# LongmaoTeamTf/deep_recommenders

Hardware: AMD Instinct MI355X
Metric: examples/sec/node DeepFM (26 sparse feats, 10M vocab, dim 64) (higher is better)
Workload: dtype f32; 1 GPU; DeepFM Criteo-shape synthetic training step (BASELINE.json configs[2]): 26 sparse + 13 dense, 10000000 vocab/field hashed on device, dim 64, DNN [256, 32]+[1] relu, sigmoid-CE, fused SGD; batch 65536 per GPU, ids uniform; tables on one GPU (66.6 GB); gemm_split=f16x2, global_batch=65536, parallelism=single, per_kernel_events=False

## Files before the change

deep_recommenders_amd/csrc/bf3_wgrad.hip:

```cpp
#ifndef DR_NT_WGRAD_GATHER
#define DR_NT_WGRAD_GATHER 0
#endif
#include "bf3_rs_core.h"

namespace {

using namespace drrs;

struct TnRsArgs {
    const float* X; int64_t ldx;
    const float* Y; int64_t ldy;
    int64_t R; int32_t F; int32_t N;
    int64_t per; int32_t split;
    float* partial; float* colsum;
    const int32_t* ids_t; const int64_t* row_base; const float* table; int32_t nf; const float* dense_pad;
    const uint32_t* x_amax; const uint32_t* x2_amax; const uint32_t* y_amax;
};

template <int GATHER, int H2 = 0>
__global__ __launch_bounds__(512, 2) void bf3_gemm_tn_rs_kernel(TnRsArgs g) {
    constexpr int NW = 8, BMF = 32 * NW, BN = 256, NT = BN / 32;
    constexpr int NPL = RS_NPL<H2>, B_PLANE = RS_B_PLANE, STAGE = RS_STAGE<H2>;
    __shared__ __attribute__((aligned(1024))) unsigned char smem[2 * STAGE];

    const int tid = threadIdx.x, lane = tid & 63;
    const int wave = __builtin_amdgcn_readfirstlane(tid >> 6);
    const int l31 = lane & 31, hi = lane >> 5;
    const int tiles_n = (g.N + BN - 1) / BN, tiles_f = (g.F + BMF - 1) / BMF;
    const int per_slice = tiles_f * tiles_n;
    const int Fp = tiles_f * BMF, Np = tiles_n * BN;
    const int lid = xcd_remap(blockIdx.x, per_slice * g.split);
    const int slice = lid / per_slice, t = lid % per_slice;
    const int f0 = (t / tiles_n) * BMF, n0 = (t % tiles_n) * BN;
    const int64_t r_begin = (int64_t)slice * g.per;
    int64_t r_end = r_begin + g.per;
    if (r_end > g.R) r_end = g.R;
    const int nk = (int)((r_end - r_begin + BK - 1) / BK);
    const bool want_cs = g.colsum != nullptr && f0 == 0;
    float h2_sx = 1.f, h2_sy = 1.f;
    if constexpr (H2) {
        float inv;
        h2_prologue(g.x_amax, g.x2_amax, g.y_amax, h2_sx, h2_sy, inv);
    }

    const int fcol = min(f0 + wave * 32 + l31, g.F - 1);
    const int ncol = min(n0 + wave * 32 + l31, g.N - 1);
    const unsigned lds0 = (unsigned)(uintptr_t)(lds_ptr_t)smem;
    const int sw = tn_img_swizzle(l31);
    unsigned b_addr[2];
#pragma unroll
    for (int s = 0; s < 2; ++s) b_addr[s] = rs_frag_addr(lds0, l31, hi, sw, s);
    unsigned char* const wrow = smem + (wave * 32 + l31) * 64;

    float xa[16], yb[16];
    const unsigned xoff = (unsigned)((16 * hi * g.ldx + fcol) * 4), yoff = (unsigned)((16 * hi * g.ldy + ncol) * 4);
    auto load_raw = [&](float (&dst)[16], const float* base, int64_t ld, unsigned voff, int64_t r0) {
        if (r0 + BK <= r_end) {
// ... 219 lines not shown
    }
}

void launch_tn_rs_reduce(const float* partial, const float* colsum, int split, int32_t F, int32_t N, int Fp, int Np, float scale,
                         float* dst, int64_t ld, float* dstb, const uint32_t* x_amax, const uint32_t* x2_amax, const uint32_t* y_amax,
                         dr_stream_t stream) {
    const bool vec = ((reinterpret_cast<uintptr_t>(partial) | reinterpret_cast<uintptr_t>(dst)) & 15) == 0 && (ld & 3) == 0;
    if (vec)
        hipLaunchKernelGGL(bf3_tn_rs_reduce_kernel<4>, dim3(F, (N + 255) / 256), dim3(64), 0, dr_s(stream), partial, colsum, split, F, N,
                           Fp, Np, scale, dst, ld, dstb, x_amax, x2_amax, y_amax);
    else
        hipLaunchKernelGGL(bf3_tn_rs_reduce_kernel<1>, dim3(F, (N + 63) / 64), dim3(64), 0, dr_s(stream), partial, colsum, split, F, N,
                           Fp, Np, scale, dst, ld, dstb, x_amax, x2_amax, y_amax);
}

void tn_rs_plan(int64_t R, int32_t F, int32_t N, int& split, int64_t& per, int& Fp, int& Np) {
    const int tf = (F + 255) / 256, tn = (N + 255) / 256;
    Fp = tf * 256;
    Np = tn * 256;
    int64_t sp = 256 / ((int64_t)tf * tn);
    const int64_t max_split = (R + 16 * BK - 1) / (16 * BK);
    if (sp > max_split) sp = max_split;
    if (sp < 1) sp = 1;
    per = ((R + sp - 1) / sp + BK - 1) / BK * BK;
    split = (int)((R + per - 1) / per);
}
}

extern "C" int64_t dr_bf3_wgrad_workspace_bytes(int64_t R, int32_t F, int32_t N) {
    if (R <= 0 || F <= 0 || N <= 0) return 0;
// ... 3 lines not shown
    return ((int64_t)split * Fp * Np + (int64_t)split * Np) * (int64_t)sizeof(float);
}

static int wgrad_impl(const float* x, int64_t ld_x, const float* dy, int64_t ld_dy, int64_t R, int32_t F, int32_t N,
                      float scale, float* dstW, int64_t ld_w, float* dstb, void* workspace, int64_t workspace_bytes,
                      dr_stream_t stream, const uint32_t* x_amax = nullptr, const uint32_t* dy_amax = nullptr) {
    if (R <= 0 || F <= 0 || N <= 0) return DR_EINVAL;
    if (!x || !dy || !dstW || !workspace || ld_x < F || ld_dy < N || ld_w < N) return DR_EINVAL;
    if (workspace_bytes < dr_bf3_wgrad_workspace_bytes(R, F, N)) return DR_EINVAL;
    int split, Fp, Np;
    int64_t per;
    tn_rs_plan(R, F, N, split, per, Fp, Np);
    float* partial = static_cast<float*>(workspace);
    float* colsum = partial + (int64_t)split * Fp * Np;
    TnRsArgs g{x, ld_x, dy, ld_dy, R, F, N, per, split, partial, dstb != nullptr ? colsum : nullptr, nullptr, nullptr, nullptr, 0, nullptr,
               x_amax, nullptr, dy_amax};
    const int grid = (Fp / 256) * (Np / 256) * split;
    if (x_amax != nullptr) hipLaunchKernelGGL((bf3_gemm_tn_rs_kernel<0, 1>), dim3(grid), dim3(512), 0, dr_s(stream), g);
    else hipLaunchKernelGGL((bf3_gemm_tn_rs_kernel<0, 0>), dim3(grid), dim3(512), 0, dr_s(stream), g);
    launch_tn_rs_reduce(partial, dstb != nullptr ? colsum : nullptr, split, F, N, Fp, Np, scale, dstW, ld_w, dstb, x_amax, nullptr, dy_amax,
                        stream);
    DR_CHECK_LAUNCH();
    return DR_OK;
}

extern "C" int dr_bf3_wgrad(const float* x, int64_t ld_x, const float* dy, int64_t ld_dy, int64_t R, int32_t F, int32_t N,
                            float scale, float* dstW, int64_t ld_w, float* dstb, void* workspace, int64_t workspace_bytes,
                            dr_stream_t stream) {
    return wgrad_impl(x, ld_x, dy, ld_dy, R, F, N, scale, dstW, ld_w, dstb, workspace, workspace_bytes, stream);
}

extern "C" int dr_h2_wgrad(const float* x, int64_t ld_x, const uint32_t* x_amax, const float* dy, int64_t ld_dy, const uint32_t* dy_amax,
                           int64_t R, int32_t F, int32_t N, float scale, float* dstW, int64_t ld_w, float* dstb, void* workspace,
                           int64_t workspace_bytes, dr_stream_t stream) {
    if (!x_amax || !dy_amax) return DR_EINVAL;
    return wgrad_impl(x, ld_x, dy, ld_dy, R, F, N, scale, dstW, ld_w, dstb, workspace, workspace_bytes, stream, x_amax, dy_amax);
}

static int wgrad_emb_impl(const int32_t* ids_t, int64_t R, int32_t nf, const int64_t* row_base, const float* table, int32_t D,
                          const float* dense_pad, const float* dy, int64_t ld_dy, int32_t F, int32_t N, float scale, float* dstW,
                          int64_t ld_w, float* dstb, void* workspace, int64_t workspace_bytes, int32_t parts, dr_stream_t stream,
                          const uint32_t* table_amax = nullptr, const uint32_t* dense_amax = nullptr, const uint32_t* dy_amax = nullptr) {
    if (R <= 0 || F <= 0 || N <= 0 || nf <= 0) return DR_EINVAL;
    if (table_amax != nullptr && (!dy_amax || (F > 64 * nf && !dense_amax))) return DR_EINVAL;
    if (D != 64 || F < 64 * nf || F > 64 * nf + 32) return DR_ESHAPE;
    if (!ids_t || !row_base || !table || !dy || !dstW || !workspace || ld_dy < N || ld_w < N) return DR_EINVAL;
    if (F > 64 * nf && !dense_pad) return DR_EINVAL;
    if (workspace_bytes < dr_bf3_wgrad_workspace_bytes(R, F, N)) return DR_EINVAL;
    int split, Fp, Np;
    int64_t per;
    tn_rs_plan(R, F, N, split, per, Fp, Np);
    float* partial = static_cast<float*>(workspace);
    float* colsum = partial + (int64_t)split * Fp * Np;
    TnRsArgs g{nullptr, 0, dy, ld_dy, R, F, N, per, split, partial, dstb != nullptr ? colsum : nullptr, ids_t, row_base, table, nf,
               F > 64 * nf ? dense_pad : nullptr, table_amax, F > 64 * nf ? dense_amax : nullptr, dy_amax};
    const int grid = (Fp / 256) * (Np / 256) * split;
    if (parts & 1) {
        if (table_amax != nullptr) hipLaunchKernelGGL((bf3_gemm_tn_rs_kernel<1, 1>), dim3(grid), dim3(512), 0, dr_s(stream), g);
        else hipLaunchKernelGGL((bf3_gemm_tn_rs_kernel<1, 0>), dim3(grid), dim3(512), 0, dr_s(stream), g);
    }
    if (parts & 2)
        launch_tn_rs_reduce(partial, dstb != nullptr ? colsum : nullptr, split, F, N, Fp, Np, scale, dstW, ld_w, dstb, table_amax,
                            F > 64 * nf ? dense_amax : nullptr, dy_amax, stream);
    DR_CHECK_LAUNCH();
    return DR_OK;
}

extern "C" int dr_bf3_wgrad_emb(const int32_t* ids_t, int64_t R, int32_t nf, const int64_t* row_base, const float* table, int32_t D,
                                const float* dense_pad, const float* dy, int64_t ld_dy, int32_t F, int32_t N, float scale, float* dstW,
                                int64_t ld_w, float* dstb, void* workspace, int64_t workspace_bytes, int32_t parts, dr_stream_t stream) {
    if (parts < 1 || parts > 3) return DR_EINVAL;
    return wgrad_emb_impl(ids_t, R, nf, row_base, table, D, dense_pad, dy, ld_dy, F, N, scale, dstW, ld_w, dstb, workspace, workspace_bytes,
                          parts, stream);
}

extern "C" int dr_h2_wgrad_emb(const int32_t* ids_t, int64_t R, int32_t nf, const int64_t* row_base, const float* table, int32_t D,
                               const uint32_t* table_amax, const float* dense_pad, const uint32_t* dense_amax, const float* dy, int64_t ld_dy,
                               const uint32_t* dy_amax, int32_t F, int32_t N, float scale, float* dstW, int64_t ld_w, float* dstb,
                               void* workspace, int64_t workspace_bytes, int32_t parts, dr_stream_t stream) {
    if (parts < 1 || parts > 3 || !table_amax || !dy_amax) return DR_EINVAL;
    return wgrad_emb_impl(ids_t, R, nf, row_base, table, D, dense_pad, dy, ld_dy, F, N, scale, dstW, ld_w, dstb, workspace, workspace_bytes,
                          parts, stream, table_amax, dense_amax, dy_amax);
}
```

deep_recommenders_amd/csrc/h2_occ.hip:

```cpp
#include "dr_common.h"
#include "rs_args.h"
#include <algorithm>
#include <cstdlib>

namespace drrs {
namespace {

typedef _Float16 f16x4 __attribute__((ext_vector_type(4)));
typedef float f32x4 __attribute__((ext_vector_type(4)));
typedef float f32x16 __attribute__((ext_vector_type(16)));
typedef unsigned u32x4 __attribute__((ext_vector_type(4)));
typedef __attribute__((address_space(3))) void* lds_ptr_t;

#define OCC_DS_READ_B128(dst, addr, off) asm volatile("ds_read_b128 %0, %1 offset:%2" : "=v"(dst) : "v"(addr), "n"(off))
#define OCC_DS_WRITE_B64(addr, val, off) asm volatile("ds_write_b64 %0, %1 offset:%2" ::"v"(addr), "v"(val), "n"(off) : "memory")
#define OCC_DS_WRITE_B32(addr, val, off) asm volatile("ds_write_b32 %0, %1 offset:%2" ::"v"(addr), "v"(val), "n"(off) : "memory")

constexpr int BM = 256, BN = 256, BK = 32;
constexpr int PLANE = 256 * 64;
constexpr int A_OFF = 0, B_OFF = 2 * PLANE, STAGE = 4 * PLANE;

struct K4Args {
    const int32_t* ids_t;
    const uint8_t* flags;
    const int64_t* row_base; int32_t F;
    float* table; float* lin_w;
    const float* lin_old_t;
    const float* sum_x; const float* d_fm_logit;
    float scale;
    float* d_concat; int64_t ld_dc;
    uint32_t* table_amax;
};

template <int EPI, int DBG = 0>
__global__ __launch_bounds__(1024) void h2_occ_nt_kernel(RsArgs g, K4Args e) {
    __shared__ __attribute__((aligned(1024))) unsigned char smem[2 * STAGE + (EPI == 8 ? 10240 : 0)];

    const int tid = threadIdx.x, lane = tid & 63;
    const int wave = __builtin_amdgcn_readfirstlane(tid >> 6);
    const int l31 = lane & 31, hi = lane >> 5;
    const int wr = wave >> 2, wc = wave & 3;

    const int tiles_n = (g.N + BN - 1) / BN;
    const int tiles_m = (int)((g.M + BM - 1) / BM);
    const int ntiles = tiles_m * tiles_n;
    const int nk = (g.K + BK - 1) / BK;
    const bool ktail = (g.K % BK) != 0;
// ... 380 lines not shown
    }
}


constexpr int PM = 128;
constexpr int PA_PLANE = PM * 64, PB_PLANE = BN * 64;
constexpr int PA_OFF = 0, PB_OFF = 2 * PA_PLANE, PSTAGE = 2 * PA_PLANE + 2 * PB_PLANE;
constexpr int P_SXP = 2 * PSTAGE;
constexpr int P_STQ = P_SXP + PM * 256;
constexpr int P_DLP = P_STQ + 8 * 2048;
constexpr int P_LOP = P_DLP + PM * 4;
constexpr int P_UIP = P_LOP + 8 * 256;
constexpr int P_LDS = P_UIP + 8 * 256;
constexpr int P_EPI_BARRIERS = 7;

__global__ __launch_bounds__(1024) void h2_occ_pp_kernel(RsArgs g, K4Args e) {
    __shared__ __attribute__((aligned(1024))) unsigned char smem[P_LDS];

    const int tid = threadIdx.x, lane = tid & 63;
    const int wave = __builtin_amdgcn_readfirstlane(tid >> 6);
    const int grp = wave >> 3, wg = wave & 7;
    const int wr = wg >> 2, wc = wg & 3;

    const int tiles_n = (g.N + BN - 1) / BN;
    const int tiles_m = (int)((g.M + PM - 1) / PM);
    const int ntiles = tiles_m * tiles_n;
    const int nk = (g.K + BK - 1) / BK;
    const bool ktail = (g.K % BK) != 0;
    const int kv4 = (g.K + 3) / 4 * 4;
    const int nb = max(nk + 1, P_EPI_BARRIERS);

// ... 260 lines not shown
#pragma unroll
            for (int a = 0; a < 2; ++a)
#pragma unroll
                for (int b = 0; b < 2; ++b)
#pragma unroll
                    for (int reg = 0; reg < 16; ++reg) acc[a][b][reg] = 0.f;
        }
        bar();
        asm volatile("s_waitcnt vmcnt(0)" ::: "memory");
        bar();
        for (int b = P_EPI_BARRIERS; b < nb; ++b) bar();
    };

    const int n = (int)blockIdx.x < ntiles ? (ntiles - 1 - (int)blockIdx.x) / (int)gridDim.x + 1 : 0;
    auto idle = [&]() __attribute__((always_inline)) { for (int b = 0; b < nb; ++b) bar(); };
    if (grp == 1) idle();
    for (int i = grp; i < n; i += 2) {
        main_loop(i);
        epilogue(i);
    }
    if (((n ^ grp) & 1) == 0) idle();
    if (e.table_amax != nullptr) {
        uint32_t m = __float_as_uint(cmax);
#pragma unroll
        for (int o = 32; o > 0; o >>= 1) m = max(m, (uint32_t)__shfl_xor((int)m, o, 64));
        if (lane == 0 && m > __hip_atomic_load(e.table_amax, __ATOMIC_RELAXED, __HIP_MEMORY_SCOPE_AGENT)) atomicMax(e.table_amax, m);
    }
}

}

// ... 25 lines not shown
    }
#endif
    if (g.mask != nullptr) hipLaunchKernelGGL((h2_occ_nt_kernel<1>), dim3(grid), dim3(1024), 0, stream, g, K4Args{});
    else if (g.accumulate) hipLaunchKernelGGL((h2_occ_nt_kernel<3>), dim3(grid), dim3(1024), 0, stream, g, K4Args{});
    else hipLaunchKernelGGL((h2_occ_nt_kernel<0>), dim3(grid), dim3(1024), 0, stream, g, K4Args{});
    DR_CHECK_LAUNCH();
    return DR_OK;
}

}

extern "C" int dr_h2_dgrad_emb_sgd(const float* dy, int64_t ld_dy, const uint32_t* dy_amax, const void* w_planes, int64_t w_ps,
                                   int64_t w_ld, const uint32_t* w_amax, int64_t M, int32_t F, int32_t K, const int32_t* ids_t,
                                   const uint8_t* unique_flags, const int64_t* row_base, float* table, float* lin_w,
                                   const float* lin_old_t, const float* sum_x, const float* d_fm_logit, float scale, float* d_concat,
                                   int64_t ld_dconcat, uint32_t* table_amax, dr_stream_t stream) {
    using namespace drrs;
    if (M < 0 || F <= 0 || F > 64 || K <= 0 || !dy_amax || !w_amax) return DR_EINVAL;
    if (M == 0) return DR_OK;
    if (!dy || !w_planes || !ids_t || !unique_flags || !row_base || !table || !sum_x || !d_fm_logit || !d_concat) return DR_EINVAL;
    if ((lin_w != nullptr) != (lin_old_t != nullptr)) return DR_EINVAL;
    if ((reinterpret_cast<uintptr_t>(dy) & 15) != 0 || (ld_dy & 3) != 0 || ld_dy < K) return DR_EINVAL;
    if ((reinterpret_cast<uintptr_t>(w_planes) & 15) != 0 || w_ld < (K + BK - 1) / BK * BK || (w_ld & 7) != 0 || (w_ps & 7) != 0) return DR_EINVAL;
    if ((reinterpret_cast<uintptr_t>(d_concat) & 15) != 0 || (ld_dconcat & 3) != 0 || ld_dconcat < 64 * (int64_t)F) return DR_EINVAL;
    if ((reinterpret_cast<uintptr_t>(table) & 15) != 0 || (reinterpret_cast<uintptr_t>(sum_x) & 15) != 0) return DR_EINVAL;
    if (2 * w_ps * 2 + (int64_t)BK * 2 * ((K + BK - 1) / BK) > 0x7fffffffll) return DR_ESHAPE;
    if ((int64_t)(BM + 8) * ld_dy * 4 + (int64_t)K * 4 > 0x7fffffffll) return DR_ESHAPE;
    RsArgs g{};
    g.A = dy; g.lda = ld_dy; g.B = static_cast<const __bf16*>(w_planes); g.b_ps = w_ps; g.b_ld = w_ld;
    g.M = M; g.N = 64 * F; g.K = K;
    g.a_amax = dy_amax; g.b_amax = w_amax;
    K4Args e{ids_t, unique_flags, row_base, F, table, lin_w, lin_old_t, sum_x, d_fm_logit, scale, d_concat, ld_dconcat, table_amax};
    static const bool overlap = [] { const char* v = getenv("DR_FUSED_K4_OVERLAP"); return !(v && v[0] == '0' && v[1] == 0); }();
    const int64_t tiles = ((M + (overlap ? PM : BM) - 1) / (overlap ? PM : BM)) * ((g.N + BN - 1) / BN);
    if (tiles > 0x7fffffff) return DR_EINVAL;
    const int grid = (int)(tiles < 256 ? tiles : 256);
#ifdef DR_OCC_ABLATE
    {
        static const int dbg = [] { const char* v = getenv("DR_OCC_DBG"); return v ? atoi(v) : 0; }();
        if (dbg == 1024 || dbg == 2048) {
            const int grid8 = (int)std::min<int64_t>(((M + BM - 1) / BM) * ((g.N + BN - 1) / BN), 256);
            if (dbg == 1024) hipLaunchKernelGGL((h2_occ_nt_kernel<8, 1024>), dim3(grid8), dim3(1024), 0, dr_s(stream), g, e);
            else hipLaunchKernelGGL((h2_occ_nt_kernel<8, 2048>), dim3(grid8), dim3(1024), 0, dr_s(stream), g, e);
            DR_CHECK_LAUNCH();
            return DR_OK;
        }
    }
#endif
    if (overlap) hipLaunchKernelGGL(h2_occ_pp_kernel, dim3(grid), dim3(1024), 0, dr_s(stream), g, e);
    else hipLaunchKernelGGL((h2_occ_nt_kernel<8>), dim3(grid), dim3(1024), 0, dr_s(stream), g, e);
    DR_CHECK_LAUNCH();
    return DR_OK;
}
```

deep_recommenders_amd/csrc/rs_args.h:

```cpp
#pragma once
#include "dr_common.h"

namespace drrs {

__device__ __forceinline__ int xcd_remap(int bid, int nwg) {
    const int q = nwg / 8, r = nwg % 8;
    const int xcd = bid % 8, idx = bid / 8;
    return (xcd < r ? xcd * (q + 1) : r * (q + 1) + (xcd - r) * q) + idx;
}

struct RsArgs {
    const float* A; int64_t lda;
    const __bf16* B; int64_t b_ps, b_ld;
    int64_t M; int32_t N; int32_t K;
    float* C; int64_t ldc;
    const float* bias; int32_t act;
    const float* mask; int64_t ld_mask;
    int32_t accumulate;
    const float* x0; const float* xin; int64_t ldx; float diag; float* prod_out;
    const float* tau; float* cand_s; int32_t* cand_c; int32_t* cand_cnt; int64_t cand_cap;
    const int64_t* pack_pos; int32_t pack_F; const float* pack_dl; const float* pack_sumx; float* pack_lin;
    const uint32_t* a_amax; const uint32_t* b_amax;
    uint32_t* c_amax;
    const float* sm_cand_prob; const int64_t* sm_cand_ids; float sm_inv_t;
// ... 1 lines not shown
    const float* sm_lse; const float* sm_w; float sm_alpha;
};

typedef _Float16 f16x8 __attribute__((ext_vector_type(8)));
typedef float f32x8 __attribute__((ext_vector_type(8)));

__device__ __forceinline__ void h2_scale_of(uint32_t amax_bits, float& s, float& inv) {
    int e = (int)((amax_bits >> 23) & 0xffu);
    e = e < 20 ? 20 : (e > 250 ? 250 : e);
    s = __uint_as_float((uint32_t)(267 - e) << 23);
    inv = __uint_as_float((uint32_t)(e - 13) << 23);
}
__device__ __forceinline__ void h2_mode_on() { __builtin_amdgcn_s_setreg(1 | (23 << 6), 1); }

int occ_nt_launch(const RsArgs& g, hipStream_t stream);

}

int dr_scores_nt_filter(const float* a, int64_t lda, const float* b, int64_t ldb, int64_t M, int32_t N, int32_t D,
                        const float* tau, float* cand_s, int32_t* cand_c, int32_t* cand_cnt, int64_t cand_cap,
                        dr_stream_t stream);
int dr_bf3_scores_filter(const float* a, int64_t lda, const void* b_planes, int64_t b_plane_stride, int64_t b_ld, int64_t M, int32_t N,
                         int32_t K, const float* tau, float* cand_s, int32_t* cand_c, int32_t* cand_cnt, int64_t cand_cap,
                         dr_stream_t stream);
int dr_h2_scores_filter(const float* a, int64_t lda, const uint32_t* a_amax, const void* b_planes, int64_t b_plane_stride, int64_t b_ld,
                        const uint32_t* b_amax, int64_t M, int32_t N, int32_t K, const float* tau, float* cand_s, int32_t* cand_c,
                        int32_t* cand_cnt, int64_t cand_cap, dr_stream_t stream);
int dr_h2_inbatch_lse(const float* q, int64_t ldq, const uint32_t* q_amax, const void* c_planes, int64_t c_ps, int64_t c_ld,
                      const uint32_t* c_amax, int64_t B, int32_t D, const float* cand_prob, const int64_t* cand_ids, float inv_t,
                      float* part_m, float* part_l, float* pos, dr_stream_t stream);
// ... 4 lines not shown
```

deep_recommenders_amd/engine.py:

```python
import math
import os
from typing import List, Optional, Sequence

import torch

from . import ops
from .ops import _pad4


_SIDE_STREAMS = {}


def _side_streams(device):
    key = str(torch.device(device))
    if key not in _SIDE_STREAMS:
        _SIDE_STREAMS[key] = (torch.cuda.Stream(device=device), torch.cuda.Stream(device=device))
    return _SIDE_STREAMS[key]


class DeepFMEngine:
    def __init__(self, num_fields: int, vocab_per_field: int, dim: int, dnn_units: Sequence[int], batch: int,
                 num_dense: int = 0, lr: float = 0.01, device="cuda", seed: int = 42, hashed: bool = True,
                 table_init_std: Optional[float] = None, lin_init_std: float = 0.0, sorted_bwd: bool = True,
                 optimizer: str = "sgd", beta1: float = 0.9, beta2: float = 0.999, eps: float = 1e-8):
# ... 141 lines not shown
            self.ev_k4 = torch.cuda.Event()
            self.ev_dw_done = torch.cuda.Event()
            self.ev_planes = torch.cuda.Event()
            self.ev_dlogit = torch.cuda.Event()
            self.ev_lin = torch.cuda.Event()
            self.ev_fwd0 = torch.cuda.Event()
            self.ev_part1 = torch.cuda.Event()
            self.ev_small = torch.cuda.Event()
            self._ev_dense = [torch.cuda.Event(), torch.cuda.Event()]
            self._dense_by_event = False
        self.lin_side = (sorted_bwd and optimizer == "sgd" and os.environ.get("DR_LIN_SIDE", "0") == "1")
        self._k4_det = not os.environ.get("DR_K4_DETERMINISTIC", "1").startswith("0")
        self.fuse_k4 = (os.environ.get("DR_FUSE_K4", "1") != "0" and self.h2 and optimizer == "sgd" and sorted_bwd and self.no_concat
                        and D == 64 and not self.lin_side and self.lin_old_t is not None
                        and self.Ws[0].shape[0] >= F * D)
        _rs = os.environ.get("DR_REDUCE_SIDE", "0")
        self.reduce_side = sorted_bwd and optimizer == "sgd" and _rs in ("1", "2")
        self.reduce_side_wgrad = self.reduce_side and _rs == "1" and not self.h2
        self._small_pending = False
        self._planes_pending = False
        self._planes_pending_l0 = False
        self._k4_fused_done = False
        self._in_train_step = False
        self._early_issued = False
        _ov = os.environ.get("DR_OVERLAP_DW", "0")
        self.overlap_dw = _ov == "1"
        if self.overlap_dw:
            self.no_concat = False
        self.concurrent = {}
        if self.overlap_dw:
# ... 448 lines not shown
                torch.cuda.current_stream().wait_event(self.ev_lin)
            self._prefetch_issue(mark)
        else:
            self._k("emb_pool_bwd", "hbm", self.alg_bytes_bwd(),
                    lambda: ops.emb_pool_bwd(self.ids, F, self.col_start, self.row_base, D, self.d_concat, self.concat,
                                             self.sum_x, self.d_logit, -lr, self.table, self.lin_w, self.lin_bias))
        if self._small_pending:
            torch.cuda.current_stream().wait_event(self.ev_small)
            self._small_pending = False
        if self.overlap_dw and not adam:
            torch.cuda.current_stream().wait_event(self.ev_dw)

    def _backward_l0_fused_k4(self, x, dy, sc, dstW, dstb, fl):
        lr = self.lr
        torch.cuda.current_stream().wait_event(self.ev_sorted)
        self._k("linear_bwd_dw_L0", "mfma", fl, lambda: self._wgrad(0, x, dy, sc, dstW, dstb))
        w_old = self.wplanes[0].w
        early = self._early_issued
        rs = self.side_r if early else self.side
        self._refresh_stream = rs
        self.ev_dw_done.record()
        with torch.cuda.stream(rs):
            rs.wait_event(self.ev_dw_done)
            self.wplanes[0].refresh()
            self.ev_planes.record(rs)
        self._planes_pending = True
        self._planes_pending_l0 = True
        mark = self._prefetch_mark()
        if early:
            self._prefetch_issue(mark)
        if not self._k4_det:
            ops.emb_snapshot_sorted_rows(self.plan, self.table, self.R, self.x_sorted)
        work = self.alg_bytes_bwd() - 4.0 * self.B * self.F * self.D + 4.0 * self.B * dy.shape[1]
        self._k("emb_pool_bwd_fused_dgrad_L0", "hbm", work,
                lambda: ops.h2_dgrad_emb_sgd(dy, self.dh0_amax, w_old, self._ids_t[self.cur], self.plan, self.row_base, self.table,
                                             self.lin_w, self.lin_old_t, self.sum_x, self.d_logit, -lr, self.d_concat, table_amax=self.tab_amax))
        k4 = lambda parts: ops.emb_pool_bwd_sorted(self.ids, self.row_base, self.plan, self.D, self.R, self.d_concat, self.d_logit, -lr,
                                                   self.table, self.lin_w, self.lin_bias, sum_x=self.sum_x, x_sorted=self.x_sorted,
                                                   parts=parts | 8, lin_old_t=self.lin_old_t, table_amax=self.tab_amax)
        self._k("emb_pool_bwd_dups", "hbm", 0, lambda: k4(1))
        self._k("emb_hot_rows_apply", "hbm", 0, lambda: k4(2))
        if not early:
            self._prefetch_issue(mark)
        self._k4_fused_done = True

    def _launch_sort(self):
        self.ev_ids.record()
        with torch.cuda.stream(self.side):
            self.side.wait_event(self.ev_ids)
            self._k("emb_sort_slots(side stream, overlapped)", "overlap", self.B * self.F * 36,
                    lambda: ops.emb_sort_slots(self.ids, self.row_base, self.R, self.plan))
# ... 82 lines not shown
```

deep_recommenders_amd/ops.py:

```python
from typing import Optional, Sequence

import torch

from . import _lib
from ._lib import check, lib, ptr, stream_ptr


def _c(t: torch.Tensor, dtype) -> torch.Tensor:
    if t.dtype != dtype:
        raise TypeError("expected %s, got %s" % (dtype, t.dtype))
    return t if t.is_contiguous() else t.contiguous()


def hash_bucket_i64(keys: torch.Tensor, col_buckets: torch.Tensor, out: Optional[torch.Tensor] = None):
    keys = _c(keys, torch.int64)
    B, C = keys.shape
    col_buckets = _c(col_buckets, torch.int64)
    assert col_buckets.numel() == C
    if out is None:
        out = torch.empty_like(keys)
    check(lib().dr_hash_bucket_i64(ptr(keys), B, C, ptr(col_buckets), ptr(out), stream_ptr()), "dr_hash_bucket_i64")
    return out


# ... 501 lines not shown
def emb_pool_bwd_sorted(ids, row_base, plan, D, num_rows, grad, d_fm_logit, scale, dst_table, dst_lin=None, dst_bias=None,
                        concat=None, sum_x=None, slot_lin_grad=None, x_sorted=None, parts=3, lin_old_t=None, table_amax=None):
    ids = _c(ids, torch.int64)
    B, F = ids.shape
    assert grad.stride(1) == 1
    assert lin_old_t is None or (lin_old_t.shape == (F, B) and lin_old_t.is_contiguous() and lin_old_t.dtype == torch.float32)
    check(lib().dr_emb_pool_bwd_sorted(ptr(ids), ptr(row_base), ptr(plan.rows), ptr(plan.slots), ptr(plan.flags),
                                       ptr(plan.dup_heads), ptr(plan.dup_count), B, F, D, int(num_rows), ptr(grad),
                                       grad.stride(0), ptr(concat), concat.stride(0) if concat is not None else 0,
                                       ptr(sum_x), ptr(d_fm_logit), ptr(slot_lin_grad), float(scale), ptr(dst_table), ptr(dst_lin),
                                       ptr(dst_bias), ptr(x_sorted), ptr(lin_old_t), int(parts), ptr(table_amax), stream_ptr()),
          "dr_emb_pool_bwd_sorted")


def h2_dgrad_emb_sgd(dy, dy_amax, w: "H2Planes", ids_t, plan, row_base, table, lin_w, lin_old_t, sum_x, d_fm_logit, scale, d_concat,
                     table_amax=None):
    F, M = ids_t.shape
    K = dy.shape[1]
    assert dy.stride(1) == 1 and d_concat.stride(1) == 1 and table.is_contiguous() and table.shape[1] == 64 and sum_x.is_contiguous()
    assert ids_t.dtype == torch.int32 and ids_t.is_contiguous() and dy.shape[0] == M and w.rows >= 64 * F
    assert (lin_w is None) == (lin_old_t is None)
    assert lin_old_t is None or (lin_old_t.shape == (F, M) and lin_old_t.is_contiguous())
    check(lib().dr_h2_dgrad_emb_sgd(ptr(dy), dy.stride(0), ptr(dy_amax), ptr(w.buf), w.plane_stride, w.ld, ptr(w.amax), M, F, K,
                                    ptr(ids_t), ptr(plan.flags), ptr(row_base), ptr(table), ptr(lin_w), ptr(lin_old_t), ptr(sum_x),
                                    ptr(d_fm_logit), float(scale), ptr(d_concat), d_concat.stride(0), ptr(table_amax), stream_ptr()),
          "dr_h2_dgrad_emb_sgd")


def emb_lin_update_unique(ids, row_base, plan, d_fm_logit, scale, dst_lin, slot_lin_grad=None):
    ids = _c(ids, torch.int64)
    B, F = ids.shape
    check(lib().dr_emb_lin_update_unique(ptr(ids), ptr(plan.flags), B, F, ptr(row_base), ptr(d_fm_logit), ptr(slot_lin_grad),
                                         float(scale), ptr(dst_lin), stream_ptr()), "dr_emb_lin_update_unique")


def adam_lr_t(lr, beta1, beta2, step):
    return lr * (1.0 - beta2 ** step) ** 0.5 / (1.0 - beta1 ** step)


def emb_pool_bwd_sorted_adam(ids, row_base, plan, D, num_rows, grad, d_fm_logit, lr_t, beta1, beta2, eps, table, m_table,
                             v_table, lin_w=None, m_lin=None, v_lin=None, concat=None, sum_x=None, slot_lin_grad=None, x_sorted=None,
# ... 658 lines not shown
        workspace.numel() * 4, int(parts), ptr(dx_amax), stream_ptr()), "dr_h2_emb_linear_tail_fwd")
    return loss, prob, d_logit, dx


def h2_wgrad(x, x_amax, dy, dy_amax, scale, dstW, dstb=None, workspace=None):
    R, F = x.shape
    N = dy.shape[1]
    assert x.stride(1) == 1 and dy.stride(1) == 1 and dstW.shape == (F, N) and dstW.stride(1) == 1 and dy.shape[0] == R
    if workspace is None:
        workspace = bf3_wgrad_workspace(R, F, N, x.device)
    check(lib().dr_h2_wgrad(ptr(x), x.stride(0), ptr(x_amax), ptr(dy), dy.stride(0), ptr(dy_amax), R, F, N, float(scale), ptr(dstW),
                            dstW.stride(0), ptr(dstb), ptr(workspace), workspace.numel() * 4, stream_ptr()), "dr_h2_wgrad")
    return dstW


def h2_wgrad_emb(ids_t, row_base, table, table_amax, dense_pad, dense_amax, dy, dy_amax, scale, dstW, dstb=None, workspace=None, parts=3):
    nf, R = ids_t.shape
    F, N = dstW.shape
    assert ids_t.dtype == torch.int32 and ids_t.is_contiguous() and dy.stride(1) == 1 and dstW.stride(1) == 1 and dy.shape == (R, N)
    assert dense_pad is None or (dense_pad.shape == (R, 32) and dense_pad.is_contiguous())
    if workspace is None:
        workspace = bf3_wgrad_workspace(R, F, N, dy.device)
    check(lib().dr_h2_wgrad_emb(ptr(ids_t), R, nf, ptr(row_base), ptr(table), table.shape[1], ptr(table_amax), ptr(dense_pad), ptr(dense_amax),
                                ptr(dy), dy.stride(0), ptr(dy_amax), F, N, float(scale), ptr(dstW), dstW.stride(0), ptr(dstb), ptr(workspace),
                                workspace.numel() * 4, int(parts), stream_ptr()), "dr_h2_wgrad_emb")
    return dstW


class H2WeightPlanes:

    def __init__(self, W, double_buffer=False):
        K, N = W.shape
        self.W = W
        self.amax = h2_record(W.device)
        self.wt = H2Planes(N, K, W.device, self.amax)
        self.w = H2Planes(K, N, W.device, self.amax)
        self._w_alt = H2Planes(K, N, W.device, h2_record(W.device)) if double_buffer else None
        self._parts = None
        self.refresh()

# ... 1161 lines not shown
```

include/dr_hotpath.h:

```cpp
#ifndef DR_HOTPATH_H
#define DR_HOTPATH_H

#include <stdint.h>

#ifdef __cplusplus
extern "C" {
#endif

#define DR_OK 0
#define DR_EINVAL (-1)
#define DR_ELAUNCH (-2)
#define DR_ESHAPE (-3)

typedef void* dr_stream_t;

const char* dr_version(void);

#define DR_GEMM_BF16X3 0
#define DR_GEMM_NATIVE_F32 1
int32_t dr_set_gemm_mode(int32_t mode);
int32_t dr_get_gemm_mode(void);

#define DR_GEMM_SPLIT_BF16X3 0
#define DR_GEMM_SPLIT_F16X2 1
// ... 250 lines not shown
                   int64_t ld_dst, const float* y_colsum, float* dstb, void* workspace, int64_t workspace_bytes,
                   dr_stream_t stream);

int dr_h2_amax(const float* src, int64_t ld, int64_t R, int32_t C, uint32_t* amax, int32_t reset, dr_stream_t stream);
int dr_h2_split(const float* src, int64_t ld_src, int64_t R, int32_t C, void* planes, int64_t plane_stride, int64_t ld_planes,
                int64_t row_offset, int64_t col_offset, int32_t transpose, const uint32_t* amax, dr_stream_t stream);
int dr_h2_refresh_weight(const float* W, int64_t ldw, int64_t K, int32_t N, void* w_planes, int64_t w_plane_stride, int64_t w_ld,
                         void* wt_planes, int64_t wt_plane_stride, int64_t wt_ld, uint32_t* amax, uint32_t* parts, dr_stream_t stream);
int dr_h2_linear_nt(const float* A, int64_t lda, const uint32_t* a_amax, const void* b_planes, int64_t b_plane_stride, int64_t b_ld,
                    const uint32_t* b_amax, int64_t M, int32_t N, int32_t K, const float* bias, int32_t act, const float* mask,
                    int64_t ld_mask, int32_t accumulate, float* C, int64_t ldc, uint32_t* c_amax, dr_stream_t stream);
int dr_h2_dgrad_emb_sgd(const float* dy, int64_t ld_dy, const uint32_t* dy_amax, const void* w_planes, int64_t w_plane_stride,
                        int64_t w_ld, const uint32_t* w_amax, int64_t M, int32_t F, int32_t K, const int32_t* ids_t,
                        const uint8_t* unique_flags, const int64_t* row_base, float* table, float* lin_w, const float* lin_old_t,
                        const float* sum_x, const float* d_fm_logit, float scale, float* d_concat, int64_t ld_dconcat,
                        uint32_t* table_amax, dr_stream_t stream);
int dr_h2_cross_fwd(const float* x0, const float* x, int64_t ld, const uint32_t* x_amax, const void* wt_planes, int64_t plane_stride,
                    int64_t ld_planes, const uint32_t* w_amax, const float* b, float diag_scale, int64_t M, int32_t Dm, float* out,
                    float* prod_out, uint32_t* out_amax, dr_stream_t stream);
int dr_h2_emb_linear_fwd(const int64_t* ids, int64_t M, int32_t F, const int64_t* row_base, int64_t field_rows_max, const float* table,
                         int32_t D, const uint32_t* table_amax, const float* lin_w, const float* lin_bias, const float* dense_pad,
                         const uint32_t* dense_amax, float* concat, int64_t ld_concat, int32_t K, const void* wt_planes,
                         int64_t plane_stride, int64_t ld_planes, const uint32_t* w_amax, int32_t N, const float* bias, int32_t act,
                         float* sum_x, float* fm_logit, float* out, int64_t ld_out, float* lin_vals_t, dr_stream_t stream);
int64_t dr_h2_emb_linear_tail_fwd_workspace_bytes(int64_t M);
int dr_h2_emb_linear_tail_fwd(const int64_t* ids, int64_t M, int32_t F, const int64_t* row_base, int64_t field_rows_max,
                              const float* table, int32_t D, const uint32_t* table_amax, const float* lin_w, const float* lin_bias,
                              const float* dense_pad, const uint32_t* dense_amax, float* concat, int64_t ld_concat, int32_t K,
                              const void* wt_planes, int64_t plane_stride, int64_t ld_planes, const uint32_t* w_amax, int32_t N,
                              const float* bias, int32_t act, float* sum_x, float* fm_logit, float* out, int64_t ld_out,
                              float* lin_vals_t, const float* W1, int64_t ld_w1, const float* b1, int32_t H, const float* w2,
                              int64_t ld_w2, const float* b2, const float* labels, int32_t loss_mode, float scale, float* dst_w1,
                              int64_t ld_dst_w1, float* dst_b1, float* dst_w2, int64_t ld_dst_w2, float* dst_b2, float* prob,
                              float* d_logit, float* d_h, int64_t ld_dh, float* dx, int64_t ld_dx, float* loss_out, void* workspace,
                              int64_t workspace_bytes, int32_t parts, uint32_t* dx_amax, dr_stream_t stream);
int dr_h2_wgrad(const float* x, int64_t ld_x, const uint32_t* x_amax, const float* dy, int64_t ld_dy, const uint32_t* dy_amax, int64_t R,
                int32_t F, int32_t N, float scale, float* dstW, int64_t ld_w, float* dstb, void* workspace, int64_t workspace_bytes,
                dr_stream_t stream);
int dr_h2_wgrad_emb(const int32_t* ids_t, int64_t R, int32_t nf, const int64_t* row_base, const float* table, int32_t D,
                    const uint32_t* table_amax, const float* dense_pad, const uint32_t* dense_amax, const float* dy, int64_t ld_dy,
                    const uint32_t* dy_amax, int32_t F, int32_t N, float scale, float* dstW, int64_t ld_w, float* dstb, void* workspace,
                    int64_t workspace_bytes, int32_t parts, dr_stream_t stream);


int dr_cin_fwd(const float* x0, const float* x, int64_t B, int32_t H0, int32_t Hk, int32_t D, const float* W,
               int32_t Fm, const float* bias, int32_t act, float* out, dr_stream_t stream);
int dr_cin_bwd(const float* x0, const float* x, int64_t B, int32_t H0, int32_t Hk, int32_t D, const float* W,
               int32_t Fm, int32_t act, const float* out, const float* d_out, float* d_x0, float* d_x, float* dW,
               float* dbias, dr_stream_t stream);

int dr_cin_pool_fwd(const float* x0, const float* x, int64_t B, int32_t H0, int32_t Hk, int32_t D, const float* W, int32_t Fm,
                    const float* bias, int32_t act, float* out, float* pooled, dr_stream_t stream);
int64_t dr_cin_pool_bwd_workspace_bytes(int64_t B, int32_t H0, int32_t Hk, int32_t D, int32_t Fm);
int dr_cin_pool_bwd(const float* x0, const float* x, int64_t B, int32_t H0, int32_t Hk, int32_t D, const float* W, int32_t Fm,
                    int32_t act, const float* out, const float* d_out, const float* d_pooled, float* d_x0, int32_t accumulate_x0,
                    float* d_x, float* dW, float* dbias, void* ws, int64_t ws_bytes, dr_stream_t stream);

// ... 148 lines not shown
```

Before: 71.65 million examples/sec.

## Fuse L0 wgrad split-K reduction into idle group of dgrad-SGD kernel

The layer-0 weight-gradient split-K reduction is moved out of its own reduce kernel and into the otherwise idle wave group of the persistent h2 dgrad/SGD kernel. That group streams partials with batched vector loads between the kernel's barriers and writes the scaled SGD update. The wgrad GEMM now exports its inverse scale factor through a small device buffer so the fused reducer can apply it. This removes one kernel launch and overlaps the reduction with dgrad work. In exchange, the weight-plane refresh is delayed until after dgrad, and the code falls back to a separate reduce when the shape limits are not met.

```diff
diff --git a/deep_recommenders_amd/csrc/bf3_wgrad.hip b/deep_recommenders_amd/csrc/bf3_wgrad.hip
--- a/deep_recommenders_amd/csrc/bf3_wgrad.hip
+++ b/deep_recommenders_amd/csrc/bf3_wgrad.hip
@@ -15,6 +15,7 @@
     float* partial; float* colsum;
     const int32_t* ids_t; const int64_t* row_base; const float* table; int32_t nf; const float* dense_pad;
     const uint32_t* x_amax; const uint32_t* x2_amax; const uint32_t* y_amax;
+    float* factor_out;
 };
 
 template <int GATHER, int H2 = 0>
@@ -41,6 +42,7 @@
     if constexpr (H2) {
         float inv;
         h2_prologue(g.x_amax, g.x2_amax, g.y_amax, h2_sx, h2_sy, inv);
+        if (g.factor_out != nullptr && blockIdx.x == 0 && tid == 0) g.factor_out[0] = inv;
     }
 
     const int fcol = min(f0 + wave * 32 + l31, g.F - 1);
@@ -290,6 +292,9 @@
                            Fp, Np, scale, dst, ld, dstb, x_amax, x2_amax, y_amax);
 }
 
+}
+
+namespace drrs {
 void tn_rs_plan(int64_t R, int32_t F, int32_t N, int& split, int64_t& per, int& Fp, int& Np) {
     const int tf = (F + 255) / 256, tn = (N + 255) / 256;
     Fp = tf * 256;
@@ -323,7 +328,7 @@
     float* partial = static_cast<float*>(workspace);
     float* colsum = partial + (int64_t)split * Fp * Np;
     TnRsArgs g{x, ld_x, dy, ld_dy, R, F, N, per, split, partial, dstb != nullptr ? colsum : nullptr, nullptr, nullptr, nullptr, 0, nullptr,
-               x_amax, nullptr, dy_amax};
+               x_amax, nullptr, dy_amax, nullptr};
     const int grid = (Fp / 256) * (Np / 256) * split;
     if (x_amax != nullptr) hipLaunchKernelGGL((bf3_gemm_tn_rs_kernel<0, 1>), dim3(grid), dim3(512), 0, dr_s(stream), g);
     else hipLaunchKernelGGL((bf3_gemm_tn_rs_kernel<0, 0>), dim3(grid), dim3(512), 0, dr_s(stream), g);
@@ -349,7 +354,8 @@
 static int wgrad_emb_impl(const int32_t* ids_t, int64_t R, int32_t nf, const int64_t* row_base, const float* table, int32_t D,
                           const float* dense_pad, const float* dy, int64_t ld_dy, int32_t F, int32_t N, float scale, float* dstW,
                           int64_t ld_w, float* dstb, void* workspace, int64_t workspace_bytes, int32_t parts, dr_stream_t stream,
-                          const uint32_t* table_amax = nullptr, const uint32_t* dense_amax = nullptr, const uint32_t* dy_amax = nullptr) {
+                          const uint32_t* table_amax = nullptr, const uint32_t* dense_amax = nullptr, const uint32_t* dy_amax = nullptr,
+                          float* factor_out = nullptr) {
     if (R <= 0 || F <= 0 || N <= 0 || nf <= 0) return DR_EINVAL;
     if (table_amax != nullptr && (!dy_amax || (F > 64 * nf && !dense_amax))) return DR_EINVAL;
     if (D != 64 || F < 64 * nf || F > 64 * nf + 32) return DR_ESHAPE;
@@ -362,7 +368,7 @@
     float* partial = static_cast<float*>(workspace);
     float* colsum = partial + (int64_t)split * Fp * Np;
     TnRsArgs g{nullptr, 0, dy, ld_dy, R, F, N, per, split, partial, dstb != nullptr ? colsum : nullptr, ids_t, row_base, table, nf,
-               F > 64 * nf ? dense_pad : nullptr, table_amax, F > 64 * nf ? dense_amax : nullptr, dy_amax};
+               F > 64 * nf ? dense_pad : nullptr, table_amax, F > 64 * nf ? dense_amax : nullptr, dy_amax, factor_out};
     const int grid = (Fp / 256) * (Np / 256) * split;
     if (parts & 1) {
         if (table_amax != nullptr) hipLaunchKernelGGL((bf3_gemm_tn_rs_kernel<1, 1>), dim3(grid), dim3(512), 0, dr_s(stream), g);
@@ -386,8 +392,8 @@
 extern "C" int dr_h2_wgrad_emb(const int32_t* ids_t, int64_t R, int32_t nf, const int64_t* row_base, const float* table, int32_t D,
                                const uint32_t* table_amax, const float* dense_pad, const uint32_t* dense_amax, const float* dy, int64_t ld_dy,
                                const uint32_t* dy_amax, int32_t F, int32_t N, float scale, float* dstW, int64_t ld_w, float* dstb,
-                               void* workspace, int64_t workspace_bytes, int32_t parts, dr_stream_t stream) {
+                               void* workspace, int64_t workspace_bytes, int32_t parts, float* factor_out, dr_stream_t stream) {
     if (parts < 1 || parts > 3 || !table_amax || !dy_amax) return DR_EINVAL;
     return wgrad_emb_impl(ids_t, R, nf, row_base, table, D, dense_pad, dy, ld_dy, F, N, scale, dstW, ld_w, dstb, workspace, workspace_bytes,
-                          parts, stream, table_amax, dense_amax, dy_amax);
-}
+                          parts, stream, table_amax, dense_amax, dy_amax, factor_out);
+}
diff --git a/deep_recommenders_amd/csrc/h2_occ.hip b/deep_recommenders_amd/csrc/h2_occ.hip
--- a/deep_recommenders_amd/csrc/h2_occ.hip
+++ b/deep_recommenders_amd/csrc/h2_occ.hip
@@ -31,6 +31,16 @@
     float* d_concat; int64_t ld_dc;
     uint32_t* table_amax;
 };
+
+struct WgJob {
+    const float* partial; const float* colsum;
+    int32_t split, F, N, Fp, Np;
+    float scale;
+    float* dstW; int64_t ld_w; float* dstb;
+    const float* inv;
+};
+constexpr int WG_BATCH = 8;
+constexpr int WG_MAX_LOADS = WG_BATCH * 6;
 
 template <int EPI, int DBG = 0>
 __global__ __launch_bounds__(1024) void h2_occ_nt_kernel(RsArgs g, K4Args e) {
@@ -441,7 +451,7 @@
 constexpr int P_LDS = P_UIP + 8 * 256;
 constexpr int P_EPI_BARRIERS = 7;
 
-__global__ __launch_bounds__(1024) void h2_occ_pp_kernel(RsArgs g, K4Args e) {
+__global__ __launch_bounds__(1024) void h2_occ_pp_kernel(RsArgs g, K4Args e, WgJob j) {
     __shared__ __attribute__((aligned(1024))) unsigned char smem[P_LDS];
 
     const int tid = threadIdx.x, lane = tid & 63;
@@ -732,7 +742,79 @@
 
     const int n = (int)blockIdx.x < ntiles ? (ntiles - 1 - (int)blockIdx.x) / (int)gridDim.x + 1 : 0;
     auto idle = [&]() __attribute__((always_inline)) { for (int b = 0; b < nb; ++b) bar(); };
-    if (grp == 1) idle();
+    auto reduce_role = [&]() __attribute__((always_inline)) {
+        int lane_r = lane;
+        asm volatile("" : "+v"(lane_r));
+        const int c4 = lane_r * 4;
+        const int rows = j.F + (j.dstb != nullptr ? 1 : 0);
+        const int np = (j.N + 255) >> 8;
+        const int wstride = (int)gridDim.x * 8;
+        const int w0 = (int)blockIdx.x * 8 + wg;
+        const int L = w0 < rows ? ((rows - 1 - w0) / wstride + 1) * np * (j.split + 1) : 0;
+        const int bsz = (L + nb - 2) / (nb - 1);
+        const float wscale = j.inv != nullptr ? j.scale * j.inv[0] : j.scale;
+        const int64_t ps = (int64_t)j.Fp * j.Np;
+        int ir = w0, ip = 0, is = 0, cr = w0, cp = 0, cs = 0;
+        int issued = 0, consumed = 0;
+        f32x4 v[WG_BATCH];
+#pragma unroll
+        for (int u = 0; u < WG_BATCH; ++u) v[u] = f32x4{0.f, 0.f, 0.f, 0.f};
+        f32x4 sum = {0.f, 0.f, 0.f, 0.f};
+        auto dst_of = [&](int r, int n) __attribute__((always_inline)) -> float* {
+            return (r < j.F ? j.dstW + (int64_t)r * j.ld_w : j.dstb) + n;
+        };
+        auto issue = [&](f32x4& d) __attribute__((always_inline)) {
+            const int n = ip * 256 + c4;
+            if (is < j.split) {
+                const float* src = (ir < j.F ? j.partial + is * ps + (int64_t)ir * j.Np : j.colsum + (int64_t)is * j.Np) + n;
+                d = *reinterpret_cast<const f32x4*>(src);
+            } else if (n < j.N) {
+                const float* p = dst_of(ir, n);
+                d[0] = p[0]; d[1] = p[1]; d[2] = p[2]; d[3] = p[3];
+            }
+            if (++is > j.split) { is = 0; if (++ip == np) { ip = 0; ir += wstride; } }
+        };
+        auto consume = [&](const f32x4& d) __attribute__((always_inline)) {
+            const int n = cp * 256 + c4;
+            if (cs < j.split) sum += d;
+            else {
+                if (n < j.N) {
+                    const float sc = cr < j.F ? wscale : j.scale;
+                    f32x4 o;
+                    o[0] = fmaf(sc, sum[0], d[0]); o[1] = fmaf(sc, sum[1], d[1]);
+                    o[2] = fmaf(sc, sum[2], d[2]); o[3] = fmaf(sc, sum[3], d[3]);
+                    float* p = dst_of(cr, n);
+                    p[0] = o[0]; p[1] = o[1]; p[2] = o[2]; p[3] = o[3];
+                }
+                sum = f32x4{0.f, 0.f, 0.f, 0.f};
+            }
+            if (++cs > j.split) { cs = 0; if (++cp == np) { cp = 0; cr += wstride; } }
+        };
+        for (int b = 0; b < nb; ++b) {
+            if (b > 0) {
+                asm volatile("s_waitcnt vmcnt(0)" : "+v"(v[0]), "+v"(v[1]), "+v"(v[2]), "+v"(v[3]), "+v"(v[4]), "+v"(v[5]), "+v"(v[6]), "+v"(v[7]) :: "memory");
+                const int c = min(bsz, L - consumed);
+#pragma unroll
+                for (int u = 0; u < WG_BATCH; ++u)
+                    if (u < c) consume(v[u]);
+                consumed += c;
+            }
+            if (b + 1 < nb) {
+                const int c = min(bsz, L - issued);
+#pragma unroll
+                for (int u = 0; u < WG_BATCH; ++u)
+                    if (u < c) issue(v[u]);
+                issued += c;
+            } else {
+                asm volatile("s_waitcnt vmcnt(0)" ::: "memory");
+            }
+            bar();
+        }
+    };
+    if (grp == 1) {
+        if (j.partial != nullptr) reduce_role();
+        else idle();
+    }
     for (int i = grp; i < n; i += 2) {
         main_loop(i);
         epilogue(i);
@@ -788,7 +870,9 @@
                                    int64_t w_ld, const uint32_t* w_amax, int64_t M, int32_t F, int32_t K, const int32_t* ids_t,
                                    const uint8_t* unique_flags, const int64_t* row_base, float* table, float* lin_w,
                                    const float* lin_old_t, const float* sum_x, const float* d_fm_logit, float scale, float* d_concat,
-                                   int64_t ld_dconcat, uint32_t* table_amax, dr_stream_t stream) {
+                                   int64_t ld_dconcat, uint32_t* table_amax, const void* wg_workspace, int64_t wg_workspace_bytes,
+                                   int32_t wg_F, float wg_scale, float* wg_dstW, int64_t wg_ld_w, float* wg_dstb, const float* wg_factor,
+                                   dr_stream_t stream) {
     using namespace drrs;
     if (M < 0 || F <= 0 || F > 64 || K <= 0 || !dy_amax || !w_amax) return DR_EINVAL;
     if (M == 0) return DR_OK;
@@ -809,6 +893,20 @@
     const int64_t tiles = ((M + (overlap ? PM : BM) - 1) / (overlap ? PM : BM)) * ((g.N + BN - 1) / BN);
     if (tiles > 0x7fffffff) return DR_EINVAL;
     const int grid = (int)(tiles < 256 ? tiles : 256);
+    WgJob j{};
+    if (wg_workspace != nullptr) {
+        if (wg_F <= 0 || !wg_dstW || wg_ld_w < K) return DR_EINVAL;
+        if (!overlap) return DR_ESHAPE;
+        int split, Fp, Np;
+        int64_t per;
+        tn_rs_plan(M, wg_F, K, split, per, Fp, Np);
+        if (wg_workspace_bytes < ((int64_t)split * Fp * Np + (int64_t)split * Np) * (int64_t)sizeof(float)) return DR_EINVAL;
+        const int64_t rows = (int64_t)wg_F + (wg_dstb != nullptr ? 1 : 0);
+        const int64_t loads = ((rows + 8 * grid - 1) / (8 * grid)) * ((K + 255) / 256) * (split + 1);
+        if ((reinterpret_cast<uintptr_t>(wg_workspace) & 15) != 0 || (K & 3) != 0 || loads > WG_MAX_LOADS) return DR_ESHAPE;
+        const float* partial = static_cast<const float*>(wg_workspace);
+        j = WgJob{partial, partial + (int64_t)split * Fp * Np, split, wg_F, K, Fp, Np, wg_scale, wg_dstW, wg_ld_w, wg_dstb, wg_factor};
+    }
 #ifdef DR_OCC_ABLATE
     {
         static const int dbg = [] { const char* v = getenv("DR_OCC_DBG"); return v ? atoi(v) : 0; }();
@@ -821,7 +919,7 @@
         }
     }
 #endif
-    if (overlap) hipLaunchKernelGGL(h2_occ_pp_kernel, dim3(grid), dim3(1024), 0, dr_s(stream), g, e);
+    if (overlap) hipLaunchKernelGGL(h2_occ_pp_kernel, dim3(grid), dim3(1024), 0, dr_s(stream), g, e, j);
     else hipLaunchKernelGGL((h2_occ_nt_kernel<8>), dim3(grid), dim3(1024), 0, dr_s(stream), g, e);
     DR_CHECK_LAUNCH();
     return DR_OK;
diff --git a/deep_recommenders_amd/csrc/rs_args.h b/deep_recommenders_amd/csrc/rs_args.h
--- a/deep_recommenders_amd/csrc/rs_args.h
+++ b/deep_recommenders_amd/csrc/rs_args.h
@@ -39,6 +39,7 @@
 __device__ __forceinline__ void h2_mode_on() { __builtin_amdgcn_s_setreg(1 | (23 << 6), 1); }
 
 int occ_nt_launch(const RsArgs& g, hipStream_t stream);
+void tn_rs_plan(int64_t R, int32_t F, int32_t N, int& split, int64_t& per, int& Fp, int& Np);
 
 }
 
diff --git a/deep_recommenders_amd/engine.py b/deep_recommenders_amd/engine.py
--- a/deep_recommenders_amd/engine.py
+++ b/deep_recommenders_amd/engine.py
@@ -179,6 +179,9 @@
         self.fuse_k4 = (os.environ.get("DR_FUSE_K4", "1") != "0" and self.h2 and optimizer == "sgd" and sorted_bwd and self.no_concat
                         and D == 64 and not self.lin_side and self.lin_old_t is not None
                         and self.Ws[0].shape[0] >= F * D)
+        self.wgrad_reduce_fused = os.environ.get("DR_WGRAD_REDUCE_FUSED", "1") != "0" and self.fuse_k4
+        self._wg_factor = torch.ones(1, dtype=torch.float32, device=self.table.device) if self.wgrad_reduce_fused else None
+        self.wgrad_reduce_fused_steps = 0
         _rs = os.environ.get("DR_REDUCE_SIDE", "0")
         self.reduce_side = sorted_bwd and optimizer == "sgd" and _rs in ("1", "2")
         self.reduce_side_wgrad = self.reduce_side and _rs == "1" and not self.h2
@@ -657,27 +660,49 @@
     def _backward_l0_fused_k4(self, x, dy, sc, dstW, dstb, fl):
         lr = self.lr
         torch.cuda.current_stream().wait_event(self.ev_sorted)
-        self._k("linear_bwd_dw_L0", "mfma", fl, lambda: self._wgrad(0, x, dy, sc, dstW, dstb))
+        fused_red = self.wgrad_reduce_fused and not self._wgrad_reduce_deferred(0)
+        wg_args = (self._ids_t[self.cur], self.row_base, self.table, self.tab_amax, self.dense_pad, self.dense_amax, dy, self.dh0_amax, sc,
+                   dstW, dstb)
+        if fused_red:
+            self._k("linear_bwd_dw_L0", "mfma", fl,
+                    lambda: ops.h2_wgrad_emb(*wg_args, workspace=self.wg_ws[0], parts=1, factor_out=self._wg_factor))
+        else:
+            self._k("linear_bwd_dw_L0", "mfma", fl, lambda: self._wgrad(0, x, dy, sc, dstW, dstb))
         w_old = self.wplanes[0].w
         early = self._early_issued
         rs = self.side_r if early else self.side
         self._refresh_stream = rs
-        self.ev_dw_done.record()
-        with torch.cuda.stream(rs):
-            rs.wait_event(self.ev_dw_done)
-            self.wplanes[0].refresh()
-            self.ev_planes.record(rs)
-        self._planes_pending = True
-        self._planes_pending_l0 = True
-        mark = self._prefetch_mark()
-        if early:
-            self._prefetch_issue(mark)
+
+        def refresh_behind_here():
+            self.ev_dw_done.record()
+            with torch.cuda.stream(rs):
+                rs.wait_event(self.ev_dw_done)
+                self.wplanes[0].refresh()
+                self.ev_planes.record(rs)
+            self._planes_pending = True
+            self._planes_pending_l0 = True
+            mark = self._prefetch_mark()
+            if early:
+                self._prefetch_issue(mark)
+            return mark
+        if not fused_red:
+            mark = refresh_behind_here()
         if not self._k4_det:
             ops.emb_snapshot_sorted_rows(self.plan, self.table, self.R, self.x_sorted)
         work = self.alg_bytes_bwd() - 4.0 * self.B * self.F * self.D + 4.0 * self.B * dy.shape[1]
-        self._k("emb_pool_bwd_fused_dgrad_L0", "hbm", work,
-                lambda: ops.h2_dgrad_emb_sgd(dy, self.dh0_amax, w_old, self._ids_t[self.cur], self.plan, self.row_base, self.table,
-                                             self.lin_w, self.lin_old_t, self.sum_x, self.d_logit, -lr, self.d_concat, table_amax=self.tab_amax))
+        dgrad = lambda job: ops.h2_dgrad_emb_sgd(dy, self.dh0_amax, w_old, self._ids_t[self.cur], self.plan, self.row_base, self.table,
+                                                 self.lin_w, self.lin_old_t, self.sum_x, self.d_logit, -lr, self.d_concat,
+                                                 table_amax=self.tab_amax, wgrad_job=job)
+
+        def dgrad_with_reduce():
+            if dgrad((self.wg_ws[0], sc, dstW, dstb, self._wg_factor)):
+                self.wgrad_reduce_fused_steps += 1
+                return
+            ops.h2_wgrad_emb(*wg_args, workspace=self.wg_ws[0], parts=2)
+            dgrad(None)
+        self._k("emb_pool_bwd_fused_dgrad_L0", "hbm", work, dgrad_with_reduce if fused_red else (lambda: dgrad(None)))
+        if fused_red:
+            mark = refresh_behind_here()
         k4 = lambda parts: ops.emb_pool_bwd_sorted(self.ids, self.row_base, self.plan, self.D, self.R, self.d_concat, self.d_logit, -lr,
                                                    self.table, self.lin_w, self.lin_bias, sum_x=self.sum_x, x_sorted=self.x_sorted,
                                                    parts=parts | 8, lin_old_t=self.lin_old_t, table_amax=self.tab_amax)
diff --git a/deep_recommenders_amd/ops.py b/deep_recommenders_amd/ops.py
--- a/deep_recommenders_amd/ops.py
+++ b/deep_recommenders_amd/ops.py
@@ -539,17 +539,28 @@
 
 
 def h2_dgrad_emb_sgd(dy, dy_amax, w: "H2Planes", ids_t, plan, row_base, table, lin_w, lin_old_t, sum_x, d_fm_logit, scale, d_concat,
-                     table_amax=None):
+                     table_amax=None, wgrad_job=None):
     F, M = ids_t.shape
     K = dy.shape[1]
     assert dy.stride(1) == 1 and d_concat.stride(1) == 1 and table.is_contiguous() and table.shape[1] == 64 and sum_x.is_contiguous()
     assert ids_t.dtype == torch.int32 and ids_t.is_contiguous() and dy.shape[0] == M and w.rows >= 64 * F
     assert (lin_w is None) == (lin_old_t is None)
     assert lin_old_t is None or (lin_old_t.shape == (F, M) and lin_old_t.is_contiguous())
-    check(lib().dr_h2_dgrad_emb_sgd(ptr(dy), dy.stride(0), ptr(dy_amax), ptr(w.buf), w.plane_stride, w.ld, ptr(w.amax), M, F, K,
-                                    ptr(ids_t), ptr(plan.flags), ptr(row_base), ptr(table), ptr(lin_w), ptr(lin_old_t), ptr(sum_x),
-                                    ptr(d_fm_logit), float(scale), ptr(d_concat), d_concat.stride(0), ptr(table_amax), stream_ptr()),
-          "dr_h2_dgrad_emb_sgd")
+    if wgrad_job is not None:
+        ws, wg_scale, dstW, dstb, factor = wgrad_job
+        assert dstW.stride(1) == 1 and dstW.shape[1] == K and ws.dtype == torch.float32 and ws.is_contiguous()
+        assert factor is None or (factor.dtype == torch.float32 and factor.numel() == 1)
+        assert dstb is None or (dstb.is_contiguous() and dstb.numel() == K)
+        job = (ptr(ws), ws.numel() * 4, dstW.shape[0], float(wg_scale), ptr(dstW), dstW.stride(0), ptr(dstb), ptr(factor))
+    else:
+        job = (None, 0, 0, 0.0, None, 0, None, None)
+    rc = lib().dr_h2_dgrad_emb_sgd(ptr(dy), dy.stride(0), ptr(dy_amax), ptr(w.buf), w.plane_stride, w.ld, ptr(w.amax), M, F, K,
+                                   ptr(ids_t), ptr(plan.flags), ptr(row_base), ptr(table), ptr(lin_w), ptr(lin_old_t), ptr(sum_x),
+                                   ptr(d_fm_logit), float(scale), ptr(d_concat), d_concat.stride(0), ptr(table_amax), *job, stream_ptr())
+    if wgrad_job is not None and rc == _lib.DR_ESHAPE:
+        return False
+    check(rc, "dr_h2_dgrad_emb_sgd")
+    return True
 
 
 def emb_lin_update_unique(ids, row_base, plan, d_fm_logit, scale, dst_lin, slot_lin_grad=None):
@@ -1238,16 +1249,18 @@
     return dstW
 
 
-def h2_wgrad_emb(ids_t, row_base, table, table_amax, dense_pad, dense_amax, dy, dy_amax, scale, dstW, dstb=None, workspace=None, parts=3):
+def h2_wgrad_emb(ids_t, row_base, table, table_amax, dense_pad, dense_amax, dy, dy_amax, scale, dstW, dstb=None, workspace=None, parts=3,
+                 factor_out=None):
     nf, R = ids_t.shape
     F, N = dstW.shape
     assert ids_t.dtype == torch.int32 and ids_t.is_contiguous() and dy.stride(1) == 1 and dstW.stride(1) == 1 and dy.shape == (R, N)
     assert dense_pad is None or (dense_pad.shape == (R, 32) and dense_pad.is_contiguous())
+    assert factor_out is None or (factor_out.dtype == torch.float32 and factor_out.numel() == 1)
     if workspace is None:
         workspace = bf3_wgrad_workspace(R, F, N, dy.device)
     check(lib().dr_h2_wgrad_emb(ptr(ids_t), R, nf, ptr(row_base), ptr(table), table.shape[1], ptr(table_amax), ptr(dense_pad), ptr(dense_amax),
                                 ptr(dy), dy.stride(0), ptr(dy_amax), F, N, float(scale), ptr(dstW), dstW.stride(0), ptr(dstb), ptr(workspace),
-                                workspace.numel() * 4, int(parts), stream_ptr()), "dr_h2_wgrad_emb")
+                                workspace.numel() * 4, int(parts), ptr(factor_out), stream_ptr()), "dr_h2_wgrad_emb")
     return dstW
 
 
diff --git a/include/dr_hotpath.h b/include/dr_hotpath.h
--- a/include/dr_hotpath.h
+++ b/include/dr_hotpath.h
@@ -288,7 +288,8 @@
                         int64_t w_ld, const uint32_t* w_amax, int64_t M, int32_t F, int32_t K, const int32_t* ids_t,
                         const uint8_t* unique_flags, const int64_t* row_base, float* table, float* lin_w, const float* lin_old_t,
                         const float* sum_x, const float* d_fm_logit, float scale, float* d_concat, int64_t ld_dconcat,
-                        uint32_t* table_amax, dr_stream_t stream);
+                        uint32_t* table_amax, const void* wg_workspace, int64_t wg_workspace_bytes, int32_t wg_F, float wg_scale,
+                        float* wg_dstW, int64_t wg_ld_w, float* wg_dstb, const float* wg_factor, dr_stream_t stream);
 int dr_h2_cross_fwd(const float* x0, const float* x, int64_t ld, const uint32_t* x_amax, const void* wt_planes, int64_t plane_stride,
                     int64_t ld_planes, const uint32_t* w_amax, const float* b, float diag_scale, int64_t M, int32_t Dm, float* out,
                     float* prod_out, uint32_t* out_amax, dr_stream_t stream);
@@ -314,7 +315,7 @@
 int dr_h2_wgrad_emb(const int32_t* ids_t, int64_t R, int32_t nf, const int64_t* row_base, const float* table, int32_t D,
                     const uint32_t* table_amax, const float* dense_pad, const uint32_t* dense_amax, const float* dy, int64_t ld_dy,
                     const uint32_t* dy_amax, int32_t F, int32_t N, float scale, float* dstW, int64_t ld_w, float* dstb, void* workspace,
-                    int64_t workspace_bytes, int32_t parts, dr_stream_t stream);
+                    int64_t workspace_bytes, int32_t parts, float* factor_out, dr_stream_t stream);
 
 
 int dr_cin_fwd(const float* x0, const float* x, int64_t B, int32_t H0, int32_t Hk, int32_t D, const float* W,
```

After: 71.97 million examples/sec, median of 6. No clear change (+0.4%).
